# TaceoLabs/co-snarks

Measured on NVIDIA H100. Metric: co-Groth16 proofs/sec (BN254, 2^20 constraints); MSM Mscalar/s, higher is better.
Workload: dtype u32x8 (256-bit Montgomery, integer)

## Files before the change

### co_snarks_b200/csrc/cs_api.cu

```cuda
#include <stdarg.h>
#include "cs_lib.cuh"

namespace cs {

std::string& last_error() {
  static thread_local std::string e;
  return e;
}
int fail(int code, const char* fmt, ...) {
  char buf[1024];
  va_list ap;
  va_start(ap, fmt);
  vsnprintf(buf, sizeof(buf), fmt, ap);
  va_end(ap);
  last_error() = buf;
  return code;
}
#if !defined(CS_EMU)
__attribute__((constructor)) static void cs_more_hw_queues() { setenv("CUDA_DEVICE_MAX_CONNECTIONS", "32", 0); }
#endif

std::atomic<uint64_t>& launch_counter() {
  static std::atomic<uint64_t> c{0};
  return c;
// ... 72 lines not shown
  CS_CUDA(cudaStreamCreateWithPriority(&ctx->wm, cudaStreamNonBlocking, prio_wm));
  CS_CUDA(cudaEventCreateWithFlags(&ctx->ev_wm, cudaEventDisableTiming));
  CS_CUDA(cudaEventCreateWithFlags(&ctx->ev_fork, cudaEventDisableTiming));
  CS_TRY(ntt_smem_optin<Bn254Fr>());
#if defined(CS_ENABLE_BLS12_381)
  CS_TRY(ntt_smem_optin<Bls381Fr>());
#endif
  *out = ctx;
  return 0;
}

void cs_ctx_destroy(cs_ctx* ctx) {
  if (!ctx) return;
  cudaSetDevice(ctx->device);
  cudaDeviceSynchronize();
  for (int i = 0; i < CS_NSIDE; i++) {
    ctx->msm_ws[i].release();
    if (ctx->side[i]) cudaStreamDestroy(ctx->side[i]);
    if (ctx->acc[i]) cudaStreamDestroy(ctx->acc[i]);
    if (ctx->ev_side[i]) cudaEventDestroy(ctx->ev_side[i]);
  }
  if (ctx->ev_fork) cudaEventDestroy(ctx->ev_fork);
  if (ctx->wm) cudaStreamDestroy(ctx->wm);
  if (ctx->ev_wm) cudaEventDestroy(ctx->ev_wm);
  if (ctx->ev_t0) cudaEventDestroy(ctx->ev_t0);
  ctx->io.release();
  ctx->prf_keys.release();
  ctx->sc_part.release();
  ctx->sc_res.release();
  if (ctx->own_stream && ctx->stream) cudaStreamDestroy(ctx->stream);
// ... 66 lines not shown
    if (f52_env < 0) { const char* e = getenv("CS_MSM_F52"); f52_env = e ? atoi(e) : 0; }
    if (f52_env) {
      const size_t ncoords = total * 2;
      CS_LAUNCH(k_msm_table_to_m260<Bn254Fq52 COMMA Bn254Fq>, ceil_div(ncoords, 128), 128, 0, ctx->stream,
                b->table.as<uint32_t>(), ncoords);
      b->m260 = true;
    }
  }
  CS_CUDA(cudaGetLastError());
  CS_CUDA(cudaStreamSynchronize(ctx->stream));
  return 0;
}

template <class Cfg, int G>
int msm_enqueue_t(cs_ctx* ctx, int slot, cudaStream_t st, const cs_bases* b, size_t offset,
                  const uint32_t* d_scalars, unsigned sstride, size_t n, int mont, int sort_slot) {
  typedef typename GroupOf<Cfg, G>::F F;
  return msm_enqueue<F, typename Cfg::FrP>(ctx->msm_ws[slot], b->table.as<Affine<F>>(), b->infmask.as<uint32_t>(), (uint32_t)b->n, b->sh,
                                           (uint32_t)offset, d_scalars, sstride, (uint32_t)n, mont, st,
                                           sort_slot >= 0 ? &ctx->msm_ws[sort_slot] : nullptr, b->m260, ctx->acc[slot]);
}

template <class Cfg, int G>
void msm_finish_t(cs_ctx* ctx, int slot, uint64_t* out_affine, int* out_inf) {
  typedef typename GroupOf<Cfg, G>::HF HF;
  const host::HXyzz<HF>* r = reinterpret_cast<const host::HXyzz<HF>*>(ctx->msm_ws[slot].h_result);
  host::HAffine<HF> a = host::haffine(*r);
  memcpy(out_affine, &a, sizeof(a));
  if (out_inf) *out_inf = a.is_inf() ? 1 : 0;
}

int msm_enqueue_dyn(cs_ctx* ctx, int slot, cudaStream_t st, const cs_bases* b, size_t offset,
                    const uint32_t* d_scalars, unsigned sstride, size_t n, int mont, int sort_slot) {
  CS_DISPATCH_CURVE(b->curve, {
    if (b->group == CS_G1) return msm_enqueue_t<Cfg, 0>(ctx, slot, st, b, offset, d_scalars, sstride, n, mont, sort_slot);
    return msm_enqueue_t<Cfg, 1>(ctx, slot, st, b, offset, d_scalars, sstride, n, mont, sort_slot);
  });
  return 0;
}
int bases_sort_compatible(cs_ctx* ctx, const cs_bases* a, const cs_bases* b, bool* out) {
  *out = false;
  if (!a || !b || a->curve != b->curve || a->n != b->n || a->sh.c != b->sh.c || a->sh.W != b->sh.W) return 0;
  const size_t words = (a->n + 31) / 32;
  std::vector<uint32_t> ma(words), mb(words);
  CS_CUDA(cudaMemcpyAsync(ma.data(), a->infmask.p, words * 4, cudaMemcpyDeviceToHost, ctx->stream));
  CS_CUDA(cudaMemcpyAsync(mb.data(), b->infmask.p, words * 4, cudaMemcpyDeviceToHost, ctx->stream));
  CS_CUDA(cudaStreamSynchronize(ctx->stream));
  *out = ma == mb;
  return 0;
}

int msm_finish_dyn(cs_ctx* ctx, int slot, const cs_bases* b, uint64_t* out_affine, int* out_inf) {
  CS_DISPATCH_CURVE(b->curve, {
    if (b->group == CS_G1) msm_finish_t<Cfg, 0>(ctx, slot, out_affine, out_inf);
    else msm_finish_t<Cfg, 1>(ctx, slot, out_affine, out_inf);
  });
  return 0;
}

}

extern "C" {

// ... 832 lines not shown
```

### co_snarks_b200/csrc/cs_groth16.cu

```cuda
#include <functional>
#include "cs_lib.cuh"
#include "cs_net.h"

using namespace cs;

struct cs_groth16_pk {
  int curve = 0;
  size_t nc = 0, ni = 0, nw = 0, n = 0;
  unsigned log_n = 0;
  DevBuf a_rowptr, a_col, a_coeff, b_rowptr, b_col, b_coeff;
  cs_bases *a_query = nullptr, *b_g1 = nullptr, *b_g2 = nullptr, *l_query = nullptr, *h_query = nullptr;
  std::vector<uint64_t> alpha_g1, beta_g1, beta_g2, delta_g1, delta_g2;
  std::vector<uint64_t> a_head, b1_head, b2_head;
  cs_domain* dom = nullptr;
  DevBuf coset_tab;
  DevBuf d_pub, d_wit, d_a, d_b, d_c, d_m1, d_m2;
  DevBuf c_rowptr, c_col, c_coeff;
  bool have_c = false;
  bool share_b_sort = false;
  cs_domain* dom_ark = nullptr;
  DevBuf coset_tab_ark, ginv_pows, vinv_over_n;
};

namespace {

template <class Cfg, int G>
struct HostGroup {
  typedef typename GroupOf<Cfg, G>::HF HF;
  typedef host::HXyzz<HF> X;
  typedef host::HAffine<HF> A;
  typedef host::HFp<typename Cfg::FrP> HR;
  static X load(const uint64_t* p) {
    A a;
    memcpy(&a, p, sizeof(a));
// ... 168 lines not shown
  else
    CS_LAUNCH(k_plain_mul_sub<FrP>, blocks, 256, 0, st, pk->d_a.as<uint32_t>(), pk->d_b.as<uint32_t>(),
              pk->d_c.as<uint32_t>(), pk->d_c.as<uint32_t>(), (size_t)n);
  if (pk->log_n) {
    CS_TRY((ntt_enqueue<FrP>(pk->d_c.as<uint32_t>(), pk->dom_ark->tw_inv.as<uint32_t>(), pk->log_n, 1, false, nullptr,
                             pk->vinv_over_n.as<uint32_t>(), st)));
    CS_LAUNCH(k_bit_reverse<FrP>, ceil_div(n, 256), 256, 0, st, pk->d_c.as<uint32_t>(), pk->log_n, 1u);
  } else {
    CS_LAUNCH(k_vec_scale_table<FrP>, 1, 32, 0, st, pk->d_c.as<uint32_t>(), pk->vinv_over_n.as<uint32_t>(), (size_t)1, 1u);
  }
  CS_LAUNCH(k_vec_scale_table<FrP>, blocks, 256, 0, st, pk->d_c.as<uint32_t>(), pk->ginv_pows.as<uint32_t>(), (size_t)n, 1u);
  CS_CUDA(cudaGetLastError());
  return 0;
}

int upload_inputs(cs_ctx* ctx, cs_groth16_pk* pk, int kind, const uint64_t* h_pub, const uint64_t* h_wit,
                  const uint64_t* h_m1, const uint64_t* h_m2) {
  const unsigned batch = kind == CS_REP3 ? 2 : 1;
  CS_TRY(upload(ctx, pk->d_pub, h_pub, pk->ni * 32));
  if (h_wit) CS_TRY(upload(ctx, pk->d_wit, h_wit, pk->nw * batch * 32));
  if (kind == CS_REP3 && h_m1) CS_TRY(upload(ctx, pk->d_m1, h_m1, pk->n * 32));
  if (kind == CS_REP3 && h_m2) CS_TRY(upload(ctx, pk->d_m2, h_m2, pk->n * 32));
  return 0;
}

template <class Cfg>
int local_phase(cs_ctx* ctx, cs_groth16_pk* pk, int kind, int party, const uint64_t* h_pub, const uint64_t* h_wit,
                const uint64_t* d_wit_in, const uint64_t* h_m1, const uint64_t* h_m2, const uint64_t* r_hs, const uint64_t* s_hs,
                uint64_t* out_a, uint64_t* out_b1, uint64_t* out_b2, uint64_t* out_l, uint64_t* out_h,
                unsigned parts = CS_PART_ALL, const cs_rep3_prf* prf = nullptr, const uint64_t* rs_mont = nullptr,
                uint64_t* out_rs_delta = nullptr, const std::function<void()>* overlap = nullptr,
                const std::function<int(const uint64_t*, const uint64_t*)>* mid = nullptr) {
  typedef HostGroup<Cfg, 0> H1;
  typedef HostGroup<Cfg, 1> H2;
  const unsigned batch = kind == CS_REP3 ? 2 : 1;
  const bool add_public = (kind == CS_PLAIN) || party == 0;
  const bool have_aux = pk->nw > 0;
  const bool do_a = parts & CS_PART_A, do_b1 = parts & CS_PART_B1, do_b2 = parts & CS_PART_B2,
             do_l = parts & CS_PART_L, do_h = parts & CS_PART_H;
  CS_CUDA(cudaSetDevice(ctx->device));
  CS_TRY(upload_inputs(ctx, pk, kind, h_pub, h_wit, do_h ? h_m1 : nullptr, do_h ? h_m2 : nullptr));
  CS_TRY(ctx_fork(ctx, 4));
  cudaStream_t wm = ctx->wm;
  CS_CUDA(cudaStreamWaitEvent(wm, ctx->ev_fork, 0));
  const uint32_t* wit = d_wit_in ? reinterpret_cast<const uint32_t*>(d_wit_in) : pk->d_wit.as<uint32_t>();
  if (do_h) {
    bool have_m1 = h_m1 != nullptr, have_m2 = h_m2 != nullptr;
    if (prf && kind == CS_REP3) {
      typedef typename Cfg::FrP FrP;
      const size_t n = pk->n;
      CS_TRY(pk->d_m1.reserve(n * 32));
      CS_TRY(pk->d_m2.reserve(n * 32));
      CS_TRY(ctx->prf_keys.reserve(64));
      CS_CUDA(cudaMemcpyAsync(ctx->prf_keys.p, prf->seed1, 32, cudaMemcpyHostToDevice, wm));
      CS_CUDA(cudaMemcpyAsync((char*)ctx->prf_keys.p + 32, prf->seed2, 32, cudaMemcpyHostToDevice, wm));
      CS_LAUNCH(k_rep3_masks<FrP>, ceil_div(n, 128), 128, 0, wm, ctx->prf_keys.as<uint32_t>(), prf->word_pos1,
                prf->word_pos2, prf->rounds, n, pk->d_m1.as<uint32_t>());
      CS_LAUNCH(k_rep3_masks<FrP>, ceil_div(n, 128), 128, 0, wm, ctx->prf_keys.as<uint32_t>(),
                prf->word_pos1 + 8 * n, prf->word_pos2 + 8 * n, prf->rounds, n, pk->d_m2.as<uint32_t>());
      have_m1 = have_m2 = true;
    }
    CS_TRY((witness_map_device<Cfg>(ctx, pk, kind, party, wit, have_m1, have_m2, wm)));
    {
      CS_SPAN("msm h_query");
      CS_TRY(msm_enqueue_dyn(ctx, 4, wm, pk->h_query, 0, pk->d_c.as<uint32_t>(), 1, pk->n, 1));
    }
  }
  if (have_aux) {
    CS_SPAN("compute A, B/G1, B/G2 in create proof with assignment + msm l_query");
    if (do_a) CS_TRY(msm_enqueue_dyn(ctx, 0, ctx->side[0], pk->a_query, pk->ni, wit, batch, pk->nw, 1));
    if (do_b1) CS_TRY(msm_enqueue_dyn(ctx, 1, ctx->side[1], pk->b_g1, pk->ni, wit, batch, pk->nw, 1));
    if (do_b2)
      CS_TRY(msm_enqueue_dyn(ctx, 2, ctx->side[2], pk->b_g2, pk->ni, wit, batch, pk->nw, 1,
                             (do_b1 && pk->share_b_sort) ? 1 : -1));
    if (do_l) CS_TRY(msm_enqueue_dyn(ctx, 3, ctx->side[3], pk->l_query, 0, wit, batch, pk->nw, 1));
  }
  CS_TRY(ctx_join(ctx, 4));
  CS_CUDA(cudaEventRecord(ctx->ev_wm, wm));
  CS_CUDA(cudaStreamWaitEvent(ctx->stream, ctx->ev_wm, 0));

  const size_t g1l = 2 * H1::HF::N, g2l = 4 * H1::HF::N;
  typename H1::X a_acc = H1::X::inf(), b1_acc = H1::X::inf();
  typename H2::X b2_acc = H2::X::inf();
  if (do_a) {
    a_acc = H1::mul(H1::load(pk->delta_g1.data()), r_hs);
    if (add_public) {
      a_acc = host::hadd(a_acc, H1::load(pk->a_head.data()));
      a_acc = host::hadd(a_acc, H1::load(pk->alpha_g1.data()));
      for (size_t k = 1; k < pk->ni; k++)
        a_acc = host::hadd(a_acc, H1::mul(H1::load(pk->a_head.data() + k * g1l), h_pub + k * 4));
    }
  }
// ... 300 lines not shown
    CS_TRY(upload(ctx, pk->c_col, d->c_col, d->c_nnz * 4));
    CS_TRY(upload(ctx, pk->c_coeff, d->c_coeff, d->c_nnz * 32));
    pk->have_c = true;
  }
  CS_CUDA(cudaStreamSynchronize(ctx->stream));
  pk->alpha_g1.assign(d->alpha_g1, d->alpha_g1 + 2 * fq);
  pk->beta_g1.assign(d->beta_g1, d->beta_g1 + 2 * fq);
  pk->beta_g2.assign(d->beta_g2, d->beta_g2 + 4 * fq);
  pk->delta_g1.assign(d->delta_g1, d->delta_g1 + 2 * fq);
  pk->delta_g2.assign(d->delta_g2, d->delta_g2 + 4 * fq);
  pk->a_head.assign(d->a_query, d->a_query + ni * 2 * fq);
  pk->b1_head.assign(d->b_g1_query, d->b_g1_query + ni * 2 * fq);
  pk->b2_head.assign(d->b_g2_query, d->b_g2_query + ni * 4 * fq);
  (void)g1b; (void)g2b;
  const int wb = d->window_bits;
  CS_TRY(cs_bases_upload(ctx, d->curve, CS_G1, d->a_query, d->a_query_len, wb, &pk->a_query));
  CS_TRY(cs_bases_upload(ctx, d->curve, CS_G1, d->b_g1_query, d->b_g1_query_len, wb, &pk->b_g1));
  CS_TRY(cs_bases_upload(ctx, d->curve, CS_G2, d->b_g2_query, d->b_g2_query_len, wb, &pk->b_g2));
  if (nw) CS_TRY(cs_bases_upload(ctx, d->curve, CS_G1, d->l_query, d->l_query_len, wb, &pk->l_query));
  CS_TRY(cs_bases_upload(ctx, d->curve, CS_G1, d->h_query, n, wb, &pk->h_query));
  {
    static int share_env = -1;
    if (share_env < 0) { const char* e = getenv("CS_SHARE_B_SORT"); share_env = e ? atoi(e) : 1; }
    if (share_env) CS_TRY(bases_sort_compatible(ctx, pk->b_g1, pk->b_g2, &pk->share_b_sort));
  }
  switch (d->curve) {
    case CS_BN254: CS_TRY(build_coset_table<Bn254Cfg>(ctx, pk.get())); break;
#if defined(CS_ENABLE_BLS12_381)
    case CS_BLS12_381: CS_TRY(build_coset_table<Bls381Cfg>(ctx, pk.get())); break;
#endif
    default: break;
  }
  *out = pk.release();
  return 0;
}

void cs_groth16_pk_free(cs_groth16_pk* pk) {
  if (!pk) return;
  DevBuf* bufs[] = {&pk->a_rowptr, &pk->a_col, &pk->a_coeff, &pk->b_rowptr, &pk->b_col, &pk->b_coeff, &pk->coset_tab,
                    &pk->d_pub, &pk->d_wit, &pk->d_a, &pk->d_b, &pk->d_c, &pk->d_m1, &pk->d_m2,
// ... 210 lines not shown
```

### co_snarks_b200/csrc/cs_lib.cuh

```cuda
#pragma once
#include <atomic>
#include <map>
#include <memory>
#include "cs_common.cuh"
#include "cs_params.cuh"
#include "cs_curve.cuh"
#include "cs_msm.cuh"
#include "cs_msm52.cuh"
#include "cs_ntt.cuh"
#include "cs_ntt8.cuh"
#include "cs_vec.cuh"
#include "cs_prf.cuh"
#include "cs_host_field.h"
#include "../../include/cosnarks_gpu.h"

namespace cs {

struct Bn254Cfg {
  typedef Bn254Fq FqP;
  typedef Bn254Fr FrP;
  static constexpr unsigned FR_BITS = 254;
  static constexpr unsigned TWO_ADICITY = 28;
};
struct Bls381Cfg {
// ... 5 lines not shown

template <class Cfg, int G> struct GroupOf;
template <class Cfg> struct GroupOf<Cfg, 0> {
  typedef Fp<typename Cfg::FqP> F;
  typedef host::HFp<typename Cfg::FqP> HF;
};
template <class Cfg> struct GroupOf<Cfg, 1> {
  typedef Fp2<typename Cfg::FqP> F;
  typedef host::HFp2<typename Cfg::FqP> HF;
};

static inline size_t fq_limbs64(int curve) { return curve == CS_BN254 ? 4 : 6; }
static inline size_t point_limbs64(int curve, int group) { return fq_limbs64(curve) * (group == CS_G1 ? 2 : 4); }

constexpr int CS_NSIDE = 5;

}

struct cs_ctx {
  int device = 0;
  cudaStream_t stream = nullptr;
  bool own_stream = false;
  cudaStream_t side[cs::CS_NSIDE] = {};
  cudaStream_t acc[cs::CS_NSIDE] = {};
  cudaStream_t wm = nullptr;
  cudaEvent_t ev_wm = nullptr;
  cudaEvent_t ev_fork = nullptr;
  cudaEvent_t ev_t0 = nullptr;
  cudaEvent_t ev_side[cs::CS_NSIDE] = {};
  cs::MsmWorkspace msm_ws[cs::CS_NSIDE];
  cs::DevBuf io;
  cs::DevBuf prf_keys;
  cs::DevBuf sc_part, sc_res;
};

struct cs_bases {
  int curve = 0, group = 0;
  size_t n = 0;
  cs::MsmShape sh{};
  cs::DevBuf table;
  cs::DevBuf infmask;
  bool m260 = false;
};

struct cs_domain {
// ... 19 lines not shown
    case CS_BN254: {                                                         \
      typedef Bn254Cfg Cfg;                                                  \
      __VA_ARGS__;                                                           \
    } break;                                                                 \
      CS_CASE_BLS(__VA_ARGS__)                                               \
    default:                                                                 \
      return cs::fail(CS_ERR_ARG, "unsupported curve id %d", (int)(curve));      \
  }


namespace cs {
std::atomic<uint64_t>& launch_counter();
int ctx_fork(cs_ctx* ctx, int nside);
int ctx_join(cs_ctx* ctx, int nside);
int msm_enqueue_dyn(cs_ctx* ctx, int slot, cudaStream_t st, const cs_bases* b, size_t offset,
                    const uint32_t* d_scalars, unsigned sstride, size_t n, int mont, int sort_slot = -1);
int bases_sort_compatible(cs_ctx* ctx, const cs_bases* a, const cs_bases* b, bool* out);
int msm_finish_dyn(cs_ctx* ctx, int slot, const cs_bases* b, uint64_t* out_affine, int* out_inf);
int ntt_run(cs_ctx* ctx, const cs_domain* d, uint32_t* d_data, unsigned batch, bool inverse_in_to_out,
            const uint32_t* d_post, cudaStream_t st);
}
```

### co_snarks_b200/csrc/cs_msm.cuh

```cuda
#pragma once
#include <stdlib.h>
#include "cs_common.cuh"
#include "cs_curve.cuh"

namespace cs {

constexpr unsigned MSM_SLICE_MAX = 64;
constexpr unsigned MSM_ORDER_BLOCK = 256;
constexpr unsigned MSM_RED_SEG = 4;
constexpr unsigned MSM_SIGN = 0x80000000u;

template <class FrP>
CS_GLOBAL void k_msm_digits(const uint32_t* __restrict__ scalars, uint32_t sstride, uint32_t n, int mont,
                            uint32_t c, uint32_t W, const uint32_t* __restrict__ infmask, uint32_t offset,
                            uint32_t* __restrict__ dig, uint32_t* __restrict__ count) {
  uint32_t i = blockIdx.x * blockDim.x + threadIdx.x;
  if (i >= n) return;
  if ((infmask[(offset + i) >> 5] >> ((offset + i) & 31)) & 1) {
    for (uint32_t w = 0; w < W; w++) dig[(size_t)w * n + i] = 0;
    return;
  }
  Fp<FrP> s;
  const uint4* src = reinterpret_cast<const uint4*>(scalars) + (size_t)i * sstride * (FrP::N / 4);
  CS_UNROLL
  for (int k = 0; k < FrP::N / 4; k++) {
    uint4 v = src[k];
    s.l[4 * k] = v.x; s.l[4 * k + 1] = v.y; s.l[4 * k + 2] = v.z; s.l[4 * k + 3] = v.w;
  }
  if (mont) s = s.from_mont();
  uint32_t lim[FrP::N + 1];
  CS_UNROLL
  for (int k = 0; k < FrP::N; k++) lim[k] = s.l[k];
  lim[FrP::N] = 0;
// ... 105 lines not shown
    start[nb1] = a + v[0]; sstart0[nb1] = b0 + v[1]; sstart1[nb1] = b1 + v[2]; sstart2[nb1] = b2 + v[3];
  }
}

static CS_GLOBAL void k_msm_scatter(const uint32_t* __restrict__ dig, uint32_t n, uint32_t nbases,
                             uint32_t offset, const uint32_t* __restrict__ start,
                             uint32_t* __restrict__ cursor, uint32_t* __restrict__ sorted) {
  uint32_t i = blockIdx.x * blockDim.x + threadIdx.x;
  uint32_t w = blockIdx.y;
  if (i >= n) return;
  uint32_t d = dig[(size_t)w * n + i];
  uint32_t b = d & ~MSM_SIGN;
  if (!b) return;
  uint32_t pos = start[b] + atomicAdd(&cursor[b], 1u);
  sorted[pos] = (w * nbases + offset + i) | (d & MSM_SIGN);
}

CS_D uint32_t find_bucket(const uint32_t* __restrict__ arr, uint32_t nb1, uint32_t s) {
  uint32_t lo = 0, hi = nb1;
  while (hi - lo > 1) {
    uint32_t mid = (lo + hi) >> 1;
    if (arr[mid] <= s) lo = mid; else hi = mid;
  }
  return lo;
}

static CS_GLOBAL void k_msm_slice_hist(const uint32_t* __restrict__ count, const uint32_t* __restrict__ sstart0,
                                       uint32_t nb1, uint32_t S, uint32_t* __restrict__ slice_len,
                                       uint32_t* __restrict__ slice_bkt, uint32_t* __restrict__ block_hist) {
  __shared__ uint32_t h[MSM_SLICE_MAX + 1];
// ... 332 lines not shown
    sorted_ev = nullptr;
    sorted_ev_made = sorted_once = false;
    dig.release(); sorted.release(); meta.release(); part0.release(); part1.release(); part2.release();
    bucket.release(); red.release(); scal.release(); result.release(); order.release();
    if (h_result) cudaFreeHost(h_result);
    h_result = nullptr;
    h_result_cap = 0;
  }
};

template <class F>
int msm_accum0_f52(const Affine<F>* table, const uint32_t* sorted, const uint32_t* count, const uint32_t* start,
                   const uint32_t* sstart0, uint32_t nb1, uint32_t S, const uint32_t* order, const uint32_t* order_b,
                   Xyzz<F>* part0, uint32_t max_s0, cudaStream_t st);

template <class F, class FrP>
int msm_enqueue(MsmWorkspace& ws, const Affine<F>* table, const uint32_t* infmask, uint32_t nbases, MsmShape sh,
                uint32_t offset,
                const uint32_t* d_scalars, uint32_t sstride, uint32_t n, int mont, cudaStream_t st,
                MsmWorkspace* sort_from = nullptr, bool table_m260 = false, cudaStream_t st_acc = nullptr) {
  const uint32_t nb1 = sh.B + 1;
  const size_t nent = (size_t)sh.W * n;
  if (nent >= (1ull << 31) || (size_t)sh.W * nbases >= (1ull << 31))
    return fail(-3, "msm: W*n = %zu exceeds 2^31 entries", nent);
  const uint32_t S = msm_slice(sh);
  const size_t max_s0 = nent / S + nb1;
  const size_t max_s1 = max_s0 / S + nb1;
  const size_t max_s2 = max_s1 / S + nb1;
  MsmWorkspace& so = sort_from ? *sort_from : ws;
  const size_t meta_words = 2 * (size_t)nb1 + 4 * ((size_t)nb1 + 1) + 4 * MSM_SCAN_MAX_BLOCKS;
  if (!sort_from) {
    CS_TRY(ws.dig.reserve(nent * 4));
    CS_TRY(ws.sorted.reserve(nent * 4));
    CS_TRY(ws.meta.reserve(meta_words * 4));
  }
  CS_TRY(ws.part0.reserve(max_s0 * sizeof(Xyzz<F>)));
  CS_TRY(ws.part1.reserve(max_s1 * sizeof(Xyzz<F>)));
  CS_TRY(ws.part2.reserve(max_s2 * sizeof(Xyzz<F>)));
  CS_TRY(ws.bucket.reserve((size_t)nb1 * sizeof(Xyzz<F>)));
  const uint32_t L = sh.B < MSM_RED_SEG ? sh.B : MSM_RED_SEG;
  const uint32_t nseg = (sh.B + L - 1) / L;
  const uint32_t fs_threads = sizeof(Xyzz<F>) > 128 ? 128 : 256;
  const uint32_t fs_blocks = nseg > 4 * fs_threads ? (nseg + fs_threads - 1) / fs_threads : 1;
  CS_TRY(ws.red.reserve(((size_t)nseg + fs_blocks) * sizeof(Xyzz<F>)));
  CS_TRY(ws.result.reserve(sizeof(Xyzz<F>)));
  const uint32_t ob = ceil_div(max_s0, MSM_ORDER_BLOCK);
  const size_t order_words = 4 * max_s0 + (size_t)ob * (MSM_SLICE_MAX + 1) + 2 * (MSM_SLICE_MAX + 1) +
                             (size_t)(MSM_SLICE_MAX + 1) * MSM_OFF_CHUNKS;
  if (!sort_from) CS_TRY(ws.order.reserve(order_words * 4));
  if (ws.h_result_cap < sizeof(Xyzz<F>)) {
    if (ws.h_result) cudaFreeHost(ws.h_result);
    CS_CUDA(cudaMallocHost(&ws.h_result, sizeof(Xyzz<F>)));
    ws.h_result_cap = sizeof(Xyzz<F>);
  }
  uint32_t* slice_len = so.order.as<uint32_t>();
  uint32_t* slice_bkt = slice_len + max_s0;
  uint32_t* order = slice_bkt + max_s0;
  uint32_t* order_b = order + max_s0;
  uint32_t* block_hist = order_b + max_s0;
  uint32_t* len_base = block_hist + (size_t)ob * (MSM_SLICE_MAX + 1);
  uint32_t* chunk_sum = len_base + 2 * (MSM_SLICE_MAX + 1);
  uint32_t* count = so.meta.as<uint32_t>();
  uint32_t* cursor = count + nb1;
  uint32_t* start = cursor + nb1;
  uint32_t* sstart0 = start + nb1 + 1;
  uint32_t* sstart1 = sstart0 + nb1 + 1;
  uint32_t* sstart2 = sstart1 + nb1 + 1;
  if (sort_from) {
    if (!sort_from->sorted_once) return fail(-1, "msm: the workspace to share a sort with has not been enqueued");
    CS_TRY(ws.mark(0, st));
    CS_CUDA(cudaStreamWaitEvent(st, sort_from->sorted_ev, 0));
    CS_TRY(ws.mark(1, st));
  } else {
    CS_TRY(ws.mark(0, st));
    CS_CUDA(cudaMemsetAsync(count, 0, 2 * (size_t)nb1 * 4, st));
    CS_LAUNCH(k_msm_digits<FrP>, ceil_div(n, 256), 256, 0, st, d_scalars, sstride, n, mont, sh.c, sh.W, infmask, offset,
              ws.dig.as<uint32_t>(), count);
    CS_TRY(ws.mark(1, st));
    {
      const uint32_t sb = ceil_div(nb1, MSM_SCAN_T);
      if (sb > MSM_SCAN_MAX_BLOCKS) return fail(-3, "msm: %u buckets exceed the scan's limit", sh.B);
      uint32_t* aux = sstart2 + nb1 + 1;
      CS_LAUNCH_SYNC(k_msm_scan1, sb, MSM_SCAN_T, 0, st, count, nb1, S, start, sstart0, sstart1, sstart2, aux);
      CS_LAUNCH(k_msm_scan2, sb, MSM_SCAN_T, 0, st, count, nb1, S, start, sstart0, sstart1, sstart2, aux);
    }
    CS_LAUNCH(k_msm_scatter, dim3(ceil_div(n, 256), sh.W), 256, 0, st, ws.dig.as<uint32_t>(), n, nbases,
              offset, start, cursor, ws.sorted.as<uint32_t>());
    CS_LAUNCH_SYNC(k_msm_slice_hist, ob, MSM_ORDER_BLOCK, 0, st, count, sstart0, nb1, S, slice_len, slice_bkt, block_hist);
    {
      const uint32_t nt = (MSM_SLICE_MAX + 1) * MSM_OFF_CHUNKS;
      CS_LAUNCH(k_msm_slice_off1, ceil_div(nt, 128), 128, 0, st, block_hist, ob, chunk_sum);
      CS_LAUNCH(k_msm_slice_off2, 1, 128, 0, st, chunk_sum, len_base);
      CS_LAUNCH(k_msm_slice_off3, ceil_div(nt, 128), 128, 0, st, block_hist, ob, chunk_sum, len_base);
    }
    CS_LAUNCH_SYNC(k_msm_slice_order, ob, MSM_ORDER_BLOCK, 0, st, slice_len, slice_bkt, (uint32_t)max_s0, sstart0, nb1,
                   block_hist, len_base, order, order_b);
    if (!ws.sorted_ev_made) {
      CS_CUDA(cudaEventCreateWithFlags(&ws.sorted_ev, cudaEventDisableTiming));
      ws.sorted_ev_made = true;
    }
    CS_CUDA(cudaEventRecord(ws.sorted_ev, st));
    ws.sorted_once = true;
  }
  CS_TRY(ws.mark(2, st));
  cudaStream_t st_main = st;
  if (st_acc) {
    if (!ws.acc_in) {
      CS_CUDA(cudaEventCreateWithFlags(&ws.acc_in, cudaEventDisableTiming));
      CS_CUDA(cudaEventCreateWithFlags(&ws.acc_out, cudaEventDisableTiming));
    }
    CS_CUDA(cudaEventRecord(ws.acc_in, st));
    CS_CUDA(cudaStreamWaitEvent(st_acc, ws.acc_in, 0));
    st = st_acc;
  }
  {
    static int minb_env = -1;
    if (minb_env < 0) { const char* e = getenv("CS_ACCUM0_MINB"); minb_env = e ? atoi(e) : 0; }
    const int minb = minb_env ? minb_env : (sizeof(Affine<F>) > 64 ? 2 : 4);
// ... 50 lines not shown
```

Measured before the change: 46.28.

## Sort witness scalars once and derive per-query bucket views by filtering

The witness-scalar bucket sort for the A, B/G1, B/G2 and L MSMs now runs once on a dedicated side stream without any infinity mask. Each query then either reuses that sort directly, reuses another query's sort when the masks match, or builds a filtered view that drops entries for infinity bases using ballot/popcount compaction. This replaces up to four independent digit/scan/scatter passes with one sort plus lighter filter passes. In exchange it adds a fifth forked stream, an extra workspace, and a serial dependency of all witness MSMs on the shared sort. The witness tables are also forced to a common window size.

```diff
diff --git a/co_snarks_b200/csrc/cs_api.cu b/co_snarks_b200/csrc/cs_api.cu
--- a/co_snarks_b200/csrc/cs_api.cu
+++ b/co_snarks_b200/csrc/cs_api.cu
@@ -110,6 +110,7 @@
   if (!ctx) return;
   cudaSetDevice(ctx->device);
   cudaDeviceSynchronize();
+  ctx->msm_ws[CS_WIT_SORT].release();
   for (int i = 0; i < CS_NSIDE; i++) {
     ctx->msm_ws[i].release();
     if (ctx->side[i]) cudaStreamDestroy(ctx->side[i]);
@@ -206,11 +207,11 @@
 
 template <class Cfg, int G>
 int msm_enqueue_t(cs_ctx* ctx, int slot, cudaStream_t st, const cs_bases* b, size_t offset,
-                  const uint32_t* d_scalars, unsigned sstride, size_t n, int mont, int sort_slot) {
+                  const uint32_t* d_scalars, unsigned sstride, size_t n, int mont, int sort_slot, bool view) {
   typedef typename GroupOf<Cfg, G>::F F;
   return msm_enqueue<F, typename Cfg::FrP>(ctx->msm_ws[slot], b->table.as<Affine<F>>(), b->infmask.as<uint32_t>(), (uint32_t)b->n, b->sh,
                                            (uint32_t)offset, d_scalars, sstride, (uint32_t)n, mont, st,
-                                           sort_slot >= 0 ? &ctx->msm_ws[sort_slot] : nullptr, b->m260, ctx->acc[slot]);
+                                           sort_slot >= 0 ? &ctx->msm_ws[sort_slot] : nullptr, view, b->m260, ctx->acc[slot]);
 }
 
 template <class Cfg, int G>
@@ -223,22 +224,19 @@
 }
 
 int msm_enqueue_dyn(cs_ctx* ctx, int slot, cudaStream_t st, const cs_bases* b, size_t offset,
-                    const uint32_t* d_scalars, unsigned sstride, size_t n, int mont, int sort_slot) {
+                    const uint32_t* d_scalars, unsigned sstride, size_t n, int mont, int sort_slot, bool view) {
   CS_DISPATCH_CURVE(b->curve, {
-    if (b->group == CS_G1) return msm_enqueue_t<Cfg, 0>(ctx, slot, st, b, offset, d_scalars, sstride, n, mont, sort_slot);
-    return msm_enqueue_t<Cfg, 1>(ctx, slot, st, b, offset, d_scalars, sstride, n, mont, sort_slot);
-  });
-  return 0;
-}
-int bases_sort_compatible(cs_ctx* ctx, const cs_bases* a, const cs_bases* b, bool* out) {
-  *out = false;
-  if (!a || !b || a->curve != b->curve || a->n != b->n || a->sh.c != b->sh.c || a->sh.W != b->sh.W) return 0;
-  const size_t words = (a->n + 31) / 32;
-  std::vector<uint32_t> ma(words), mb(words);
-  CS_CUDA(cudaMemcpyAsync(ma.data(), a->infmask.p, words * 4, cudaMemcpyDeviceToHost, ctx->stream));
-  CS_CUDA(cudaMemcpyAsync(mb.data(), b->infmask.p, words * 4, cudaMemcpyDeviceToHost, ctx->stream));
-  CS_CUDA(cudaStreamSynchronize(ctx->stream));
-  *out = ma == mb;
+    if (b->group == CS_G1) return msm_enqueue_t<Cfg, 0>(ctx, slot, st, b, offset, d_scalars, sstride, n, mont, sort_slot, view);
+    return msm_enqueue_t<Cfg, 1>(ctx, slot, st, b, offset, d_scalars, sstride, n, mont, sort_slot, view);
+  });
+  return 0;
+}
+int msm_sort_shared_dyn(cs_ctx* ctx, int slot, cudaStream_t st, const cs_bases* b, const uint32_t* d_scalars,
+                        unsigned sstride, size_t n, int mont) {
+  CS_DISPATCH_CURVE(b->curve, {
+    return msm_sort<typename Cfg::FrP>(ctx->msm_ws[slot], nullptr, (uint32_t)n, b->sh, 0, d_scalars, sstride, (uint32_t)n,
+                                       mont, st);
+  });
   return 0;
 }
 
diff --git a/co_snarks_b200/csrc/cs_groth16.cu b/co_snarks_b200/csrc/cs_groth16.cu
--- a/co_snarks_b200/csrc/cs_groth16.cu
+++ b/co_snarks_b200/csrc/cs_groth16.cu
@@ -17,7 +17,7 @@
   DevBuf d_pub, d_wit, d_a, d_b, d_c, d_m1, d_m2;
   DevBuf c_rowptr, c_col, c_coeff;
   bool have_c = false;
-  bool share_b_sort = false;
+  int wit_src[4] = {0, 1, 2, 3};
   cs_domain* dom_ark = nullptr;
   DevBuf coset_tab_ark, ginv_pows, vinv_over_n;
 };
@@ -216,6 +216,39 @@
   return 0;
 }
 
+int plan_witness_views(cs_ctx* ctx, cs_groth16_pk* pk) {
+  const size_t ni = pk->ni, nw = pk->nw;
+  if (!nw) return 0;
+  const cs_bases* q[4] = {pk->a_query, pk->b_g1, pk->b_g2, pk->l_query};
+  const size_t off[4] = {ni, ni, ni, 0};
+  std::vector<uint8_t> inf[4];
+  for (int j = 0; j < 4; j++) {
+    if (q[j]->sh.c != q[0]->sh.c || q[j]->sh.W != q[0]->sh.W)
+      return fail(CS_ERR_STATE, "cs_groth16_pk_create: the witness MSMs' tables differ in window shape");
+    std::vector<uint32_t> words((q[j]->n + 31) / 32);
+    CS_CUDA(cudaMemcpyAsync(words.data(), q[j]->infmask.p, words.size() * 4, cudaMemcpyDeviceToHost, ctx->stream));
+    CS_CUDA(cudaStreamSynchronize(ctx->stream));
+    inf[j].resize(nw);
+    bool any = false;
+    for (size_t i = 0; i < nw; i++) {
+      const size_t k = off[j] + i;
+      inf[j][i] = (words[k >> 5] >> (k & 31)) & 1;
+      any = any || inf[j][i];
+    }
+    pk->wit_src[j] = j;
+    if (q[j]->n == nw && off[j] == 0 && !any) {
+      pk->wit_src[j] = -1;
+      continue;
+    }
+    for (int k = 0; k < j; k++)
+      if (pk->wit_src[k] == k && q[k]->n == q[j]->n && off[k] == off[j] && inf[k] == inf[j]) {
+        pk->wit_src[j] = k;
+        break;
+      }
+  }
+  return 0;
+}
+
 int upload_inputs(cs_ctx* ctx, cs_groth16_pk* pk, int kind, const uint64_t* h_pub, const uint64_t* h_wit,
                   const uint64_t* h_m1, const uint64_t* h_m2) {
   const unsigned batch = kind == CS_REP3 ? 2 : 1;
@@ -242,7 +275,7 @@
              do_l = parts & CS_PART_L, do_h = parts & CS_PART_H;
   CS_CUDA(cudaSetDevice(ctx->device));
   CS_TRY(upload_inputs(ctx, pk, kind, h_pub, h_wit, do_h ? h_m1 : nullptr, do_h ? h_m2 : nullptr));
-  CS_TRY(ctx_fork(ctx, 4));
+  CS_TRY(ctx_fork(ctx, 5));
   cudaStream_t wm = ctx->wm;
   CS_CUDA(cudaStreamWaitEvent(wm, ctx->ev_fork, 0));
   const uint32_t* wit = d_wit_in ? reinterpret_cast<const uint32_t*>(d_wit_in) : pk->d_wit.as<uint32_t>();
@@ -270,14 +303,20 @@
   }
   if (have_aux) {
     CS_SPAN("compute A, B/G1, B/G2 in create proof with assignment + msm l_query");
-    if (do_a) CS_TRY(msm_enqueue_dyn(ctx, 0, ctx->side[0], pk->a_query, pk->ni, wit, batch, pk->nw, 1));
-    if (do_b1) CS_TRY(msm_enqueue_dyn(ctx, 1, ctx->side[1], pk->b_g1, pk->ni, wit, batch, pk->nw, 1));
-    if (do_b2)
-      CS_TRY(msm_enqueue_dyn(ctx, 2, ctx->side[2], pk->b_g2, pk->ni, wit, batch, pk->nw, 1,
-                             (do_b1 && pk->share_b_sort) ? 1 : -1));
-    if (do_l) CS_TRY(msm_enqueue_dyn(ctx, 3, ctx->side[3], pk->l_query, 0, wit, batch, pk->nw, 1));
-  }
-  CS_TRY(ctx_join(ctx, 4));
+    const unsigned part[4] = {CS_PART_A, CS_PART_B1, CS_PART_B2, CS_PART_L};
+    const cs_bases* q[4] = {pk->a_query, pk->b_g1, pk->b_g2, pk->l_query};
+    const size_t off[4] = {pk->ni, pk->ni, pk->ni, 0};
+    if (do_a || do_b1 || do_b2 || do_l)
+      CS_TRY(msm_sort_shared_dyn(ctx, CS_WIT_SORT, ctx->side[4], pk->a_query, wit, batch, pk->nw, 1));
+    for (int j = 0; j < 4; j++) {
+      if (!(parts & part[j])) continue;
+      int src = pk->wit_src[j];
+      if (src >= 0 && !(parts & part[src])) src = j;
+      const int sort_slot = src < 0 || src == j ? CS_WIT_SORT : src;
+      CS_TRY(msm_enqueue_dyn(ctx, j, ctx->side[j], q[j], off[j], wit, batch, pk->nw, 1, sort_slot, src == j));
+    }
+  }
+  CS_TRY(ctx_join(ctx, 5));
   CS_CUDA(cudaEventRecord(ctx->ev_wm, wm));
   CS_CUDA(cudaStreamWaitEvent(ctx->stream, ctx->ev_wm, 0));
 
@@ -608,16 +647,14 @@
   pk->b2_head.assign(d->b_g2_query, d->b_g2_query + ni * 4 * fq);
   (void)g1b; (void)g2b;
   const int wb = d->window_bits;
-  CS_TRY(cs_bases_upload(ctx, d->curve, CS_G1, d->a_query, d->a_query_len, wb, &pk->a_query));
-  CS_TRY(cs_bases_upload(ctx, d->curve, CS_G1, d->b_g1_query, d->b_g1_query_len, wb, &pk->b_g1));
-  CS_TRY(cs_bases_upload(ctx, d->curve, CS_G2, d->b_g2_query, d->b_g2_query_len, wb, &pk->b_g2));
-  if (nw) CS_TRY(cs_bases_upload(ctx, d->curve, CS_G1, d->l_query, d->l_query_len, wb, &pk->l_query));
+  int wwb = wb;
+  if (!wwb) CS_DISPATCH_CURVE(d->curve, { wwb = (int)msm_auto_window(nw, Cfg::FR_BITS); });
+  CS_TRY(cs_bases_upload(ctx, d->curve, CS_G1, d->a_query, d->a_query_len, wwb, &pk->a_query));
+  CS_TRY(cs_bases_upload(ctx, d->curve, CS_G1, d->b_g1_query, d->b_g1_query_len, wwb, &pk->b_g1));
+  CS_TRY(cs_bases_upload(ctx, d->curve, CS_G2, d->b_g2_query, d->b_g2_query_len, wwb, &pk->b_g2));
+  if (nw) CS_TRY(cs_bases_upload(ctx, d->curve, CS_G1, d->l_query, d->l_query_len, wwb, &pk->l_query));
   CS_TRY(cs_bases_upload(ctx, d->curve, CS_G1, d->h_query, n, wb, &pk->h_query));
-  {
-    static int share_env = -1;
-    if (share_env < 0) { const char* e = getenv("CS_SHARE_B_SORT"); share_env = e ? atoi(e) : 1; }
-    if (share_env) CS_TRY(bases_sort_compatible(ctx, pk->b_g1, pk->b_g2, &pk->share_b_sort));
-  }
+  CS_TRY(plan_witness_views(ctx, pk.get()));
   switch (d->curve) {
     case CS_BN254: CS_TRY(build_coset_table<Bn254Cfg>(ctx, pk.get())); break;
 #if defined(CS_ENABLE_BLS12_381)
diff --git a/co_snarks_b200/csrc/cs_lib.cuh b/co_snarks_b200/csrc/cs_lib.cuh
--- a/co_snarks_b200/csrc/cs_lib.cuh
+++ b/co_snarks_b200/csrc/cs_lib.cuh
@@ -43,6 +43,7 @@
 static inline size_t point_limbs64(int curve, int group) { return fq_limbs64(curve) * (group == CS_G1 ? 2 : 4); }
 
 constexpr int CS_NSIDE = 5;
+constexpr int CS_WIT_SORT = CS_NSIDE;
 
 }
 
@@ -57,7 +58,7 @@
   cudaEvent_t ev_fork = nullptr;
   cudaEvent_t ev_t0 = nullptr;
   cudaEvent_t ev_side[cs::CS_NSIDE] = {};
-  cs::MsmWorkspace msm_ws[cs::CS_NSIDE];
+  cs::MsmWorkspace msm_ws[cs::CS_NSIDE + 1];
   cs::DevBuf io;
   cs::DevBuf prf_keys;
   cs::DevBuf sc_part, sc_res;
@@ -107,8 +108,9 @@
 int ctx_fork(cs_ctx* ctx, int nside);
 int ctx_join(cs_ctx* ctx, int nside);
 int msm_enqueue_dyn(cs_ctx* ctx, int slot, cudaStream_t st, const cs_bases* b, size_t offset,
-                    const uint32_t* d_scalars, unsigned sstride, size_t n, int mont, int sort_slot = -1);
-int bases_sort_compatible(cs_ctx* ctx, const cs_bases* a, const cs_bases* b, bool* out);
+                    const uint32_t* d_scalars, unsigned sstride, size_t n, int mont, int sort_slot = -1, bool view = false);
+int msm_sort_shared_dyn(cs_ctx* ctx, int slot, cudaStream_t st, const cs_bases* b, const uint32_t* d_scalars,
+                        unsigned sstride, size_t n, int mont);
 int msm_finish_dyn(cs_ctx* ctx, int slot, const cs_bases* b, uint64_t* out_affine, int* out_inf);
 int ntt_run(cs_ctx* ctx, const cs_domain* d, uint32_t* d_data, unsigned batch, bool inverse_in_to_out,
             const uint32_t* d_post, cudaStream_t st);
diff --git a/co_snarks_b200/csrc/cs_msm.cuh b/co_snarks_b200/csrc/cs_msm.cuh
--- a/co_snarks_b200/csrc/cs_msm.cuh
+++ b/co_snarks_b200/csrc/cs_msm.cuh
@@ -16,7 +16,7 @@
                             uint32_t* __restrict__ dig, uint32_t* __restrict__ count) {
   uint32_t i = blockIdx.x * blockDim.x + threadIdx.x;
   if (i >= n) return;
-  if ((infmask[(offset + i) >> 5] >> ((offset + i) & 31)) & 1) {
+  if (infmask && ((infmask[(offset + i) >> 5] >> ((offset + i) & 31)) & 1)) {
     for (uint32_t w = 0; w < W; w++) dig[(size_t)w * n + i] = 0;
     return;
   }
@@ -152,6 +152,103 @@
   if (!b) return;
   uint32_t pos = start[b] + atomicAdd(&cursor[b], 1u);
   sorted[pos] = (w * nbases + offset + i) | (d & MSM_SIGN);
+}
+
+constexpr unsigned MSM_VIEW_T = 256;
+constexpr unsigned MSM_VIEW_WORDS = MSM_VIEW_T / 32;
+
+CS_D uint32_t popc32(uint32_t x) {
+#if defined(CS_EMU)
+  return (uint32_t)__builtin_popcount(x);
+#else
+  return __popc(x);
+#endif
+}
+CS_D uint32_t warp_bits(bool pred) {
+#if defined(CS_EMU)
+  uint32_t x = pred ? 1u << (threadIdx.x & 31) : 0u;
+  for (uint32_t d = 16; d > 0; d >>= 1) x += __shfl_xor_sync(0xffffffffu, x, d);
+  return x;
+#else
+  return __ballot_sync(0xffffffffu, pred);
+#endif
+}
+
+static CS_GLOBAL void k_msm_view_flags(const uint32_t* __restrict__ sorted, const uint32_t* __restrict__ src_start,
+                                       uint32_t nb1, uint32_t n, const uint32_t* __restrict__ infmask, uint32_t offset,
+                                       uint32_t* __restrict__ keep, uint32_t* __restrict__ blk_cnt) {
+  __shared__ uint32_t cnt[MSM_VIEW_WORDS];
+  const uint32_t t = threadIdx.x;
+  const uint32_t p = blockIdx.x * MSM_VIEW_T + t;
+  bool k = false;
+  if (p < src_start[nb1]) {
+    const uint32_t i = (sorted[p] & ~MSM_SIGN) % n;
+    k = !((infmask[(offset + i) >> 5] >> ((offset + i) & 31)) & 1);
+  }
+  const uint32_t bits = warp_bits(k);
+  if ((t & 31) == 0) {
+    keep[(size_t)blockIdx.x * MSM_VIEW_WORDS + (t >> 5)] = bits;
+    cnt[t >> 5] = popc32(bits);
+  }
+  __syncthreads();
+  if (t == 0) {
+    uint32_t c = 0;
+    for (uint32_t w = 0; w < MSM_VIEW_WORDS; w++) c += cnt[w];
+    blk_cnt[blockIdx.x] = c;
+  }
+}
+
+static CS_GLOBAL void k_msm_view_scan(const uint32_t* __restrict__ blk_cnt, uint32_t nblk, uint32_t* __restrict__ blk_off) {
+  __shared__ uint32_t sm[MSM_SCAN_T];
+  const uint32_t t = threadIdx.x, T = blockDim.x;
+  const uint32_t per = (nblk + T - 1) / T;
+  const uint32_t lo = t * per < nblk ? t * per : nblk, hi = lo + per < nblk ? lo + per : nblk;
+  uint32_t s = 0;
+  for (uint32_t b = lo; b < hi; b++) s += blk_cnt[b];
+  sm[t] = s;
+  __syncthreads();
+  for (uint32_t d = 1; d < T; d <<= 1) {
+    const uint32_t v = t >= d ? sm[t - d] : 0;
+    __syncthreads();
+    sm[t] += v;
+    __syncthreads();
+  }
+  uint32_t run = sm[t] - s;
+  for (uint32_t b = lo; b < hi; b++) {
+    const uint32_t c = blk_cnt[b];
+    blk_off[b] = run;
+    run += c;
+  }
+  if (t == T - 1) blk_off[nblk] = run;
+}
+
+CS_D uint32_t view_kept_before(uint32_t p, const uint32_t* __restrict__ keep, const uint32_t* __restrict__ blk_off) {
+  const uint32_t blk = p / MSM_VIEW_T;
+  uint32_t r = blk_off[blk];
+  for (uint32_t w = blk * MSM_VIEW_WORDS; w < (p >> 5); w++) r += popc32(keep[w]);
+  if (p & 31) r += popc32(keep[p >> 5] & ((1u << (p & 31)) - 1));
+  return r;
+}
+
+static CS_GLOBAL void k_msm_view_counts(const uint32_t* __restrict__ src_start, uint32_t nb1, const uint32_t* __restrict__ keep,
+                                        const uint32_t* __restrict__ blk_off, uint32_t* __restrict__ count) {
+  const uint32_t b = blockIdx.x * blockDim.x + threadIdx.x;
+  if (b >= nb1) return;
+  count[b] = b ? view_kept_before(src_start[b + 1], keep, blk_off) - view_kept_before(src_start[b], keep, blk_off) : 0;
+}
+
+static CS_GLOBAL void k_msm_view_scatter(const uint32_t* __restrict__ sorted, uint32_t n, uint32_t nbases, uint32_t offset,
+                                         const uint32_t* __restrict__ keep, const uint32_t* __restrict__ blk_off,
+                                         uint32_t* __restrict__ out) {
+  const uint32_t t = threadIdx.x;
+  const uint32_t* kb = keep + (size_t)blockIdx.x * MSM_VIEW_WORDS;
+  const uint32_t word = kb[t >> 5];
+  if (!((word >> (t & 31)) & 1)) return;
+  uint32_t pos = blk_off[blockIdx.x] + popc32(word & ((1u << (t & 31)) - 1));
+  for (uint32_t k = 0; k < (t >> 5); k++) pos += popc32(kb[k]);
+  const uint32_t e = sorted[blockIdx.x * MSM_VIEW_T + t];
+  const uint32_t v = e & ~MSM_SIGN, w = v / n, i = v - w * n;
+  out[pos] = (w * nbases + offset + i) | (e & MSM_SIGN);
 }
 
 CS_D uint32_t find_bucket(const uint32_t* __restrict__ arr, uint32_t nb1, uint32_t s) {
@@ -514,26 +611,129 @@
                    const uint32_t* sstart0, uint32_t nb1, uint32_t S, const uint32_t* order, const uint32_t* order_b,
                    Xyzz<F>* part0, uint32_t max_s0, cudaStream_t st);
 
+struct MsmSizes {
+  uint32_t nb1, S, ob;
+  size_t nent, max_s0, max_s1, max_s2;
+  MsmSizes(const MsmShape& sh, uint32_t n) {
+    nb1 = sh.B + 1;
+    nent = (size_t)sh.W * n;
+    S = msm_slice(sh);
+    max_s0 = nent / S + nb1;
+    max_s1 = max_s0 / S + nb1;
+    max_s2 = max_s1 / S + nb1;
+    ob = ceil_div(max_s0, MSM_ORDER_BLOCK);
+  }
+  size_t meta_words() const { return 2 * (size_t)nb1 + 4 * ((size_t)nb1 + 1) + 4 * MSM_SCAN_MAX_BLOCKS; }
+  size_t order_words() const {
+    return 4 * max_s0 + (size_t)ob * (MSM_SLICE_MAX + 1) + 2 * (MSM_SLICE_MAX + 1) + (size_t)(MSM_SLICE_MAX + 1) * MSM_OFF_CHUNKS;
+  }
+};
+struct MsmSortBufs {
+  uint32_t *count, *cursor, *start, *sstart0, *sstart1, *sstart2, *aux;
+  uint32_t *slice_len, *slice_bkt, *order, *order_b, *block_hist, *len_base, *chunk_sum;
+  MsmSortBufs(const MsmWorkspace& w, const MsmSizes& z) {
+    count = w.meta.as<uint32_t>();
+    cursor = count + z.nb1;
+    start = cursor + z.nb1;
+    sstart0 = start + z.nb1 + 1;
+    sstart1 = sstart0 + z.nb1 + 1;
+    sstart2 = sstart1 + z.nb1 + 1;
+    aux = sstart2 + z.nb1 + 1;
+    slice_len = w.order.as<uint32_t>();
+    slice_bkt = slice_len + z.max_s0;
+    order = slice_bkt + z.max_s0;
+    order_b = order + z.max_s0;
+    block_hist = order_b + z.max_s0;
+    len_base = block_hist + (size_t)z.ob * (MSM_SLICE_MAX + 1);
+    chunk_sum = len_base + 2 * (MSM_SLICE_MAX + 1);
+  }
+};
+
+static inline int msm_check_limits(const MsmShape& sh, uint32_t n, uint32_t nbases) {
+  const size_t nent = (size_t)sh.W * n;
+  if (nent >= (1ull << 31) || (size_t)sh.W * nbases >= (1ull << 31))
+    return fail(-3, "msm: W*n = %zu exceeds 2^31 entries", nent);
+  return 0;
+}
+
+static inline int msm_scan(const MsmSortBufs& q, const MsmSizes& z, uint32_t B, cudaStream_t st) {
+  const uint32_t sb = ceil_div(z.nb1, MSM_SCAN_T);
+  if (sb > MSM_SCAN_MAX_BLOCKS) return fail(-3, "msm: %u buckets exceed the scan's limit", B);
+  CS_LAUNCH_SYNC(k_msm_scan1, sb, MSM_SCAN_T, 0, st, q.count, z.nb1, z.S, q.start, q.sstart0, q.sstart1, q.sstart2, q.aux);
+  CS_LAUNCH(k_msm_scan2, sb, MSM_SCAN_T, 0, st, q.count, z.nb1, z.S, q.start, q.sstart0, q.sstart1, q.sstart2, q.aux);
+  return 0;
+}
+
+static inline int msm_slice_order(MsmWorkspace& ws, const MsmSortBufs& q, const MsmSizes& z, cudaStream_t st) {
+  CS_LAUNCH_SYNC(k_msm_slice_hist, z.ob, MSM_ORDER_BLOCK, 0, st, q.count, q.sstart0, z.nb1, z.S, q.slice_len, q.slice_bkt,
+                 q.block_hist);
+  const uint32_t nt = (MSM_SLICE_MAX + 1) * MSM_OFF_CHUNKS;
+  CS_LAUNCH(k_msm_slice_off1, ceil_div(nt, 128), 128, 0, st, q.block_hist, z.ob, q.chunk_sum);
+  CS_LAUNCH(k_msm_slice_off2, 1, 128, 0, st, q.chunk_sum, q.len_base);
+  CS_LAUNCH(k_msm_slice_off3, ceil_div(nt, 128), 128, 0, st, q.block_hist, z.ob, q.chunk_sum, q.len_base);
+  CS_LAUNCH_SYNC(k_msm_slice_order, z.ob, MSM_ORDER_BLOCK, 0, st, q.slice_len, q.slice_bkt, (uint32_t)z.max_s0, q.sstart0,
+                 z.nb1, q.block_hist, q.len_base, q.order, q.order_b);
+  if (!ws.sorted_ev_made) {
+    CS_CUDA(cudaEventCreateWithFlags(&ws.sorted_ev, cudaEventDisableTiming));
+    ws.sorted_ev_made = true;
+  }
+  CS_CUDA(cudaEventRecord(ws.sorted_ev, st));
+  ws.sorted_once = true;
+  return 0;
+}
+
+template <class FrP>
+int msm_sort(MsmWorkspace& ws, const uint32_t* infmask, uint32_t nbases, MsmShape sh, uint32_t offset,
+             const uint32_t* d_scalars, uint32_t sstride, uint32_t n, int mont, cudaStream_t st) {
+  CS_TRY(msm_check_limits(sh, n, nbases));
+  const MsmSizes z(sh, n);
+  CS_TRY(ws.dig.reserve(z.nent * 4));
+  CS_TRY(ws.sorted.reserve(z.nent * 4));
+  CS_TRY(ws.meta.reserve(z.meta_words() * 4));
+  CS_TRY(ws.order.reserve(z.order_words() * 4));
+  const MsmSortBufs q(ws, z);
+  CS_TRY(ws.mark(0, st));
+  CS_CUDA(cudaMemsetAsync(q.count, 0, 2 * (size_t)z.nb1 * 4, st));
+  CS_LAUNCH(k_msm_digits<FrP>, ceil_div(n, 256), 256, 0, st, d_scalars, sstride, n, mont, sh.c, sh.W, infmask, offset,
+            ws.dig.as<uint32_t>(), q.count);
+  CS_TRY(ws.mark(1, st));
+  CS_TRY(msm_scan(q, z, sh.B, st));
+  CS_LAUNCH(k_msm_scatter, dim3(ceil_div(n, 256), sh.W), 256, 0, st, ws.dig.as<uint32_t>(), n, nbases, offset, q.start,
+            q.cursor, ws.sorted.as<uint32_t>());
+  return msm_slice_order(ws, q, z, st);
+}
+
+static inline int msm_view(MsmWorkspace& ws, const MsmWorkspace& src, const uint32_t* infmask, uint32_t nbases,
+                           MsmShape sh, uint32_t offset, uint32_t n, cudaStream_t st) {
+  const MsmSizes z(sh, n);
+  const uint32_t nblk = ceil_div(z.nent, MSM_VIEW_T);
+  CS_TRY(ws.dig.reserve(((size_t)nblk * MSM_VIEW_WORDS + 2 * (size_t)nblk + 1) * 4));
+  CS_TRY(ws.sorted.reserve(z.nent * 4));
+  CS_TRY(ws.meta.reserve(z.meta_words() * 4));
+  CS_TRY(ws.order.reserve(z.order_words() * 4));
+  const MsmSortBufs q(ws, z), s(src, z);
+  uint32_t* keep = ws.dig.as<uint32_t>();
+  uint32_t* blk_cnt = keep + (size_t)nblk * MSM_VIEW_WORDS;
+  uint32_t* blk_off = blk_cnt + nblk;
+  const uint32_t* src_sorted = src.sorted.as<uint32_t>();
+  CS_LAUNCH_SYNC(k_msm_view_flags, nblk, MSM_VIEW_T, 0, st, src_sorted, s.start, z.nb1, n, infmask, offset, keep, blk_cnt);
+  CS_LAUNCH_SYNC(k_msm_view_scan, 1, MSM_SCAN_T, 0, st, blk_cnt, nblk, blk_off);
+  CS_LAUNCH(k_msm_view_counts, ceil_div(z.nb1, 256), 256, 0, st, s.start, z.nb1, keep, blk_off, q.count);
+  CS_LAUNCH(k_msm_view_scatter, nblk, MSM_VIEW_T, 0, st, src_sorted, n, nbases, offset, keep, blk_off,
+            ws.sorted.as<uint32_t>());
+  CS_TRY(msm_scan(q, z, sh.B, st));
+  return msm_slice_order(ws, q, z, st);
+}
+
 template <class F, class FrP>
 int msm_enqueue(MsmWorkspace& ws, const Affine<F>* table, const uint32_t* infmask, uint32_t nbases, MsmShape sh,
                 uint32_t offset,
                 const uint32_t* d_scalars, uint32_t sstride, uint32_t n, int mont, cudaStream_t st,
-                MsmWorkspace* sort_from = nullptr, bool table_m260 = false, cudaStream_t st_acc = nullptr) {
-  const uint32_t nb1 = sh.B + 1;
-  const size_t nent = (size_t)sh.W * n;
-  if (nent >= (1ull << 31) || (size_t)sh.W * nbases >= (1ull << 31))
-    return fail(-3, "msm: W*n = %zu exceeds 2^31 entries", nent);
-  const uint32_t S = msm_slice(sh);
-  const size_t max_s0 = nent / S + nb1;
-  const size_t max_s1 = max_s0 / S + nb1;
-  const size_t max_s2 = max_s1 / S + nb1;
-  MsmWorkspace& so = sort_from ? *sort_from : ws;
-  const size_t meta_words = 2 * (size_t)nb1 + 4 * ((size_t)nb1 + 1) + 4 * MSM_SCAN_MAX_BLOCKS;
-  if (!sort_from) {
-    CS_TRY(ws.dig.reserve(nent * 4));
-    CS_TRY(ws.sorted.reserve(nent * 4));
-    CS_TRY(ws.meta.reserve(meta_words * 4));
-  }
+                MsmWorkspace* sort_from = nullptr, bool view = false, bool table_m260 = false, cudaStream_t st_acc = nullptr) {
+  CS_TRY(msm_check_limits(sh, n, nbases));
+  const MsmSizes z(sh, n);
+  const uint32_t nb1 = z.nb1, S = z.S;
+  const size_t max_s0 = z.max_s0, max_s1 = z.max_s1, max_s2 = z.max_s2;
   CS_TRY(ws.part0.reserve(max_s0 * sizeof(Xyzz<F>)));
   CS_TRY(ws.part1.reserve(max_s1 * sizeof(Xyzz<F>)));
   CS_TRY(ws.part2.reserve(max_s2 * sizeof(Xyzz<F>)));
@@ -544,64 +744,24 @@
   const uint32_t fs_blocks = nseg > 4 * fs_threads ? (nseg + fs_threads - 1) / fs_threads : 1;
   CS_TRY(ws.red.reserve(((size_t)nseg + fs_blocks) * sizeof(Xyzz<F>)));
   CS_TRY(ws.result.reserve(sizeof(Xyzz<F>)));
-  const uint32_t ob = ceil_div(max_s0, MSM_ORDER_BLOCK);
-  const size_t order_words = 4 * max_s0 + (size_t)ob * (MSM_SLICE_MAX + 1) + 2 * (MSM_SLICE_MAX + 1) +
-                             (size_t)(MSM_SLICE_MAX + 1) * MSM_OFF_CHUNKS;
-  if (!sort_from) CS_TRY(ws.order.reserve(order_words * 4));
   if (ws.h_result_cap < sizeof(Xyzz<F>)) {
     if (ws.h_result) cudaFreeHost(ws.h_result);
     CS_CUDA(cudaMallocHost(&ws.h_result, sizeof(Xyzz<F>)));
     ws.h_result_cap = sizeof(Xyzz<F>);
   }
-  uint32_t* slice_len = so.order.as<uint32_t>();
-  uint32_t* slice_bkt = slice_len + max_s0;
-  uint32_t* order = slice_bkt + max_s0;
-  uint32_t* order_b = order + max_s0;
-  uint32_t* block_hist = order_b + max_s0;
-  uint32_t* len_base = block_hist + (size_t)ob * (MSM_SLICE_MAX + 1);
-  uint32_t* chunk_sum = len_base + 2 * (MSM_SLICE_MAX + 1);
-  uint32_t* count = so.meta.as<uint32_t>();
-  uint32_t* cursor = count + nb1;
-  uint32_t* start = cursor + nb1;
-  uint32_t* sstart0 = start + nb1 + 1;
-  uint32_t* sstart1 = sstart0 + nb1 + 1;
-  uint32_t* sstart2 = sstart1 + nb1 + 1;
   if (sort_from) {
     if (!sort_from->sorted_once) return fail(-1, "msm: the workspace to share a sort with has not been enqueued");
     CS_TRY(ws.mark(0, st));
     CS_CUDA(cudaStreamWaitEvent(st, sort_from->sorted_ev, 0));
     CS_TRY(ws.mark(1, st));
+    if (view) CS_TRY(msm_view(ws, *sort_from, infmask, nbases, sh, offset, n, st));
   } else {
-    CS_TRY(ws.mark(0, st));
-    CS_CUDA(cudaMemsetAsync(count, 0, 2 * (size_t)nb1 * 4, st));
-    CS_LAUNCH(k_msm_digits<FrP>, ceil_div(n, 256), 256, 0, st, d_scalars, sstride, n, mont, sh.c, sh.W, infmask, offset,
-              ws.dig.as<uint32_t>(), count);
-    CS_TRY(ws.mark(1, st));
-    {
-      const uint32_t sb = ceil_div(nb1, MSM_SCAN_T);
-      if (sb > MSM_SCAN_MAX_BLOCKS) return fail(-3, "msm: %u buckets exceed the scan's limit", sh.B);
-      uint32_t* aux = sstart2 + nb1 + 1;
-      CS_LAUNCH_SYNC(k_msm_scan1, sb, MSM_SCAN_T, 0, st, count, nb1, S, start, sstart0, sstart1, sstart2, aux);
-      CS_LAUNCH(k_msm_scan2, sb, MSM_SCAN_T, 0, st, count, nb1, S, start, sstart0, sstart1, sstart2, aux);
-    }
-    CS_LAUNCH(k_msm_scatter, dim3(ceil_div(n, 256), sh.W), 256, 0, st, ws.dig.as<uint32_t>(), n, nbases,
-              offset, start, cursor, ws.sorted.as<uint32_t>());
-    CS_LAUNCH_SYNC(k_msm_slice_hist, ob, MSM_ORDER_BLOCK, 0, st, count, sstart0, nb1, S, slice_len, slice_bkt, block_hist);
-    {
-      const uint32_t nt = (MSM_SLICE_MAX + 1) * MSM_OFF_CHUNKS;
-      CS_LAUNCH(k_msm_slice_off1, ceil_div(nt, 128), 128, 0, st, block_hist, ob, chunk_sum);
-      CS_LAUNCH(k_msm_slice_off2, 1, 128, 0, st, chunk_sum, len_base);
-      CS_LAUNCH(k_msm_slice_off3, ceil_div(nt, 128), 128, 0, st, block_hist, ob, chunk_sum, len_base);
-    }
-    CS_LAUNCH_SYNC(k_msm_slice_order, ob, MSM_ORDER_BLOCK, 0, st, slice_len, slice_bkt, (uint32_t)max_s0, sstart0, nb1,
-                   block_hist, len_base, order, order_b);
-    if (!ws.sorted_ev_made) {
-      CS_CUDA(cudaEventCreateWithFlags(&ws.sorted_ev, cudaEventDisableTiming));
-      ws.sorted_ev_made = true;
-    }
-    CS_CUDA(cudaEventRecord(ws.sorted_ev, st));
-    ws.sorted_once = true;
-  }
+    CS_TRY(msm_sort<FrP>(ws, infmask, nbases, sh, offset, d_scalars, sstride, n, mont, st));
+  }
+  MsmWorkspace& so = sort_from && !view ? *sort_from : ws;
+  const MsmSortBufs q(so, z);
+  const uint32_t *count = q.count, *start = q.start, *sstart0 = q.sstart0, *sstart1 = q.sstart1, *sstart2 = q.sstart2;
+  const uint32_t *order = q.order, *order_b = q.order_b;
   CS_TRY(ws.mark(2, st));
   cudaStream_t st_main = st;
   if (st_acc) {
```

New measurement: 47.71 (median of 6 runs). +3.1%, better.
